# invesalius/invesalius3

Measured on AMD Instinct MI355X. Metric: Mvoxel/s segmentation + Mtriangles/s marching-cubes, 512^3 int16, 1/2/4/8 GPU, higher is better.
Workload: dtype i16; 1 GPU; configs[1]: 512x512x512 int16 per GPU, threshold(226..3071) + 26-neighbour region-grow + marching-cubes(mask@127); global_voxels=134217728, parallelism=z-slab x1, collectives=none, overlap=none

## Files before the change

### include/ivx.h

```cpp
#ifndef IVX_H
#define IVX_H
#include <stddef.h>
#include <stdint.h>

#ifdef __cplusplus
extern "C" {
#endif

#define IVX_OK 0
#define IVX_EINVAL (-1)
#define IVX_ERANGE (-2)
#define IVX_ENOMEM (-3)
#define IVX_EDOM (-4)
#define IVX_EHIP (-5)
#define IVX_ESTALE (-6)

#define IVX_U8 0
#define IVX_I16 1
#define IVX_F64 2
#define IVX_U16 3
#define IVX_F32 4
#define IVX_I32 5
#define IVX_I64 6
#define IVX_I8 7
// ... 366 lines not shown
int ivx_dev_flood_or_planes(const ivx_flood_plan *p, const uint64_t *cand, uint64_t *reached, int64_t z_a,
                            const uint64_t *plane_a, int64_t z_b, const uint64_t *plane_b, void *scratch, int *changed,
                            void *stream);
int ivx_dev_flood_or_planes_dev(const ivx_flood_plan *p, const uint64_t *cand, uint64_t *reached, int64_t z_a,
                                const uint64_t *plane_a, int64_t z_b, const uint64_t *plane_b, void *scratch,
                                uint32_t *changed_dev, void *stream);
int ivx_dev_flood_or_planes_acc(const ivx_flood_plan *p, const uint64_t *cand, uint64_t *reached, int64_t z_a,
                                const uint64_t *plane_a, int64_t z_b, const uint64_t *plane_b, void *scratch,
                                uint32_t *changed_dev, void *stream);
int ivx_dev_flood_apply(const ivx_flood_plan *p, const uint64_t *reached, int dtype, void *target,
                        double fill, void *stream);
int ivx_dev_flood_apply_levels(const ivx_flood_plan *p, const uint64_t *reached, const uint64_t *inside_bits, uint8_t *mask,
                               int v_in, int v_sel, void *stream);
int ivx_dev_mask_from_planes(const ivx_flood_plan *p, const uint64_t *inside_bits, const uint64_t *reached, uint8_t *mask,
                             int v_in, int v_sel, void *stream);
int ivx_dev_flood_apply2(const ivx_flood_plan *p, const uint64_t *reached, uint8_t *out, int fill, uint8_t *mask,
                         int select, void *stream);
int ivx_dev_flood_count(const ivx_flood_plan *p, const uint64_t *reached, int64_t *count, void *stream);
int ivx_flood_edges_bytes(const ivx_flood_plan *p, size_t *nbytes);
int ivx_dev_flood_edges_auto(const ivx_flood_plan *p, const int16_t *data, const uint8_t *out, float pfrac, int fill,
                             uint64_t *edges, void *stream);
int ivx_dev_flood_seed_forced(const ivx_flood_plan *p, const int64_t *seeds_xyz, int64_t nseeds, uint64_t *cand,
                              uint64_t *reached, void *scratch, void *stream);
int ivx_dev_flood_run_edges(const ivx_flood_plan *p, const uint64_t *edges, uint64_t *reached, void *scratch, int *rounds,
                            void *stream);
int ivx_floodfill(int dtype, const void *data, const int64_t shape[3], const int64_t strides[3], int64_t x, int64_t y,
                  int64_t z, double v, int fill, uint8_t *out, const int64_t out_strides[3]);
int ivx_floodfill_auto_threshold(const int16_t *data, const int64_t shape[3], const int64_t strides[3],
                                 const int64_t *seeds_xyz, int64_t nseeds, float pfrac, int fill, uint8_t *out,
                                 const int64_t out_strides[3]);
// ... 257 lines not shown
```

### invesalius3_amd/_lib.py

```python
from __future__ import annotations

import ctypes
import os

import numpy as np

_HERE = os.path.dirname(os.path.abspath(__file__))
LIB_PATH = os.environ.get("IVX_LIB_PATH") or os.path.join(_HERE, "libivx.so")

IVX_OK, IVX_EINVAL, IVX_ERANGE, IVX_ENOMEM, IVX_EDOM, IVX_EHIP, IVX_ESTALE = 0, -1, -2, -3, -4, -5, -6
U8, I16, F64, U16, F32, I32, I64, I8 = 0, 1, 2, 3, 4, 5, 6, 7
DT = {np.dtype(np.uint8): U8, np.dtype(np.int16): I16, np.dtype(np.float64): F64, np.dtype(np.uint16): U16, np.dtype(np.float32): F32, np.dtype(np.int32): I32,
      np.dtype(np.int64): I64}
MIP_MAX, MIP_MIN, MIP_MEAN, MIP_SUM = 0, 1, 2, 3

c_i64 = ctypes.c_int64
c_vp = ctypes.c_void_p


class McParams(ctypes.Structure):
    _fields_ = [
        ("dtype", ctypes.c_int32), ("pad_xy", ctypes.c_int32), ("pad_bottom", ctypes.c_int32),
        ("pad_top", ctypes.c_int32), ("vtk_pz", ctypes.c_int32), ("niso", ctypes.c_int32),
        ("nz", c_i64), ("ny", c_i64), ("nx", c_i64), ("roi_start", c_i64),
        ("pad_value", ctypes.c_double), ("spacing", ctypes.c_double * 3), ("iso", ctypes.c_double * 2),
    ]


class FloodPlan(ctypes.Structure):
    _fields_ = [("dz", c_i64), ("dy", c_i64), ("dx", c_i64), ("wx", c_i64), ("strct_bits", ctypes.c_uint32)]


class VolrenParams(ctypes.Structure):
    _fields_ = [
        ("width", ctypes.c_int32), ("height", ctypes.c_int32), ("mip", ctypes.c_int32), ("shade", ctypes.c_int32),
        ("skip", ctypes.c_int32), ("n_table", ctypes.c_int32), ("out_u8", ctypes.c_int32), ("clip", ctypes.c_int32),
        ("origin", ctypes.c_double * 3), ("du", ctypes.c_double * 3), ("dv", ctypes.c_double * 3),
        ("dir", ctypes.c_double * 3), ("spacing", ctypes.c_double * 3), ("dt", ctypes.c_double),
        ("ambient", ctypes.c_double), ("diffuse", ctypes.c_double), ("specular", ctypes.c_double),
        ("specular_power", ctypes.c_double), ("background", ctypes.c_double * 3), ("clip_normal", ctypes.c_double * 3),
        ("clip_origin", ctypes.c_double * 3),
    ]


ROI_ELLIPSE, ROI_POLYGON, ROI_MAX_POINTS, ROI_RECORD_BYTES = 0, 1, 2048, 40
# ... 18 lines not shown
    i64p = ctypes.POINTER(c_i64)
    for name, args in (("ivx_host_register", [c_vp, sz, u64p]), ("ivx_host_touch", [u64]), ("ivx_host_touch_range", [u64, sz, sz]),
                       ("ivx_host_release", [u64]), ("ivx_host_stats", [u64, u64p]), ("ivx_host_count", [u64p]),
                       ("ivx_host_set_check", [ctypes.c_int]), ("ivx_transfer_stats", [u64p]),
                       ("ivx_upload_strided", [c_vp, c_vp, i64p, i64p, sz]), ("ivx_download_strided", [c_vp, i64p, i64p, c_vp, sz]),
                       ("ivx_image_ranges_bytes", [c_i64, c_i64, c_i64, ctypes.POINTER(sz)]),
                       ("ivx_dev_image_ranges_i16", [c_vp, c_i64, c_i64, c_i64, c_vp, c_vp]),
                       ("ivx_dev_threshold_i16_bits_ranges", [c_vp, c_i64, c_i64, c_i64, ctypes.c_int, ctypes.c_int, c_vp, c_vp, c_vp,
                                                              ctypes.c_int, c_vp]),
                       ("ivx_dev_threshold_i16_plane", [c_vp, c_i64, c_i64, c_i64, ctypes.c_int, ctypes.c_int, c_vp, c_vp]),
                       ("ivx_dev_threshold_i16_plane_ranges", [c_vp, c_i64, c_i64, c_i64, ctypes.c_int, ctypes.c_int, c_vp, c_vp,
                                                               ctypes.c_int, c_vp]),
                       ("ivx_dev_mask_from_planes", [ctypes.POINTER(FloodPlan), c_vp, c_vp, c_vp, ctypes.c_int, ctypes.c_int, c_vp]),
                       ("ivx_dev_flood_candidates_ranges", [ctypes.POINTER(FloodPlan), c_vp, ctypes.c_double, ctypes.c_double, c_vp,
                                                            ctypes.c_int, ctypes.c_double, c_vp, c_vp, c_vp]),
                       ("ivx_dev_image_flip", [c_vp, c_i64, c_i64, c_i64, sz, ctypes.c_int, c_vp]),
                       ("ivx_image_flip", [c_vp, i64p, i64p, sz, ctypes.c_int]),
                       ("ivx_dev_image_swap_axes", [c_vp, c_i64, c_i64, c_i64, sz, ctypes.c_int, ctypes.c_int, c_vp, c_vp]),
                       ("ivx_image_swap_axes", [c_vp, i64p, i64p, sz, ctypes.c_int, ctypes.c_int, c_vp, i64p]),
                       ("ivx_image_tilt_scratch_bytes", [c_i64, c_i64, c_i64, ctypes.POINTER(sz)]),
                       ("ivx_dev_image_fix_gantry_tilt", [c_vp, c_i64, c_i64, c_i64, c_vp, c_vp, sz, c_vp, c_vp]),
                       ("ivx_image_fix_gantry_tilt", [c_vp, i64p, i64p, c_vp, c_vp]),
                       ("ivx_host_zero", [c_vp, sz]), ("ivx_host_register_zero", [c_vp, sz, u64p]),
                       ("ivx_slice_show_tables_bytes", [ctypes.c_int, ctypes.POINTER(sz)]),
                       ("ivx_dev_slice_show", [c_vp, c_i64, c_i64] * 3 + [c_i64, c_i64, c_vp, c_vp, c_vp, c_vp]),
                       ("ivx_slice_show", [c_vp, c_i64, c_i64] * 3 + [c_i64, c_i64, c_vp, c_vp, c_vp]),
                       ("ivx_mask_snapshot_header_bytes", [c_i64, ctypes.POINTER(sz)]),
                       ("ivx_dev_mask_snapshot_scan", [c_vp, c_i64, c_vp, i64p, c_vp]),
                       ("ivx_dev_mask_snapshot_pack", [c_vp, c_i64, c_vp, c_vp, c_i64, c_vp]),
                       ("ivx_dev_mask_snapshot_restore", [c_vp, c_i64, c_vp, c_vp, c_i64, c_i64, c_vp, c_vp]),
# ... 127 lines not shown
```

### invesalius3_amd/csrc/k_flood.hip

```cpp
#include <math.h>
#include <map>
#include <mutex>
#include <stdlib.h>

#include "flood_tiles.h"
#include "words_from_records.h"

namespace {

constexpr int NT = TY * TZ;
constexpr int HY = TY + 2, HZ = TZ + 2;
constexpr int BATCH = 8;
constexpr int SUB = 1;
constexpr unsigned int CLOSED = 0x40u;

template <typename T> __device__ __forceinline__ double as_double(T v) { return (double)v; }

template <typename T, int BAR>
__global__ __launch_bounds__(256) void k_flood_candidates16(const short8_t *__restrict__ data,
                                                            const uint4 *__restrict__ bar, int64_t nchunks, double t0,
                                                            double t1, double fill, uint16_t *__restrict__ cand) {
    const int64_t stride = (int64_t)gridDim.x * blockDim.x;
    const int lo = (int)ceil(t0 < -70000.0 ? -70000.0 : t0), hi = (int)floor(t1 > 70000.0 ? 70000.0 : t1);
    const unsigned fb = (unsigned)(uint8_t)fill;
// ... 946 lines not shown
                auto blend = [&](unsigned int old, unsigned int bits4) {
                    const unsigned int sel = ((bits4 & 1u) * 0xffu) | ((bits4 >> 1 & 1u) * 0xff00u) |
                                             ((bits4 >> 2 & 1u) * 0xff0000u) | ((bits4 >> 3 & 1u) * 0xff000000u);
                    return (old & ~sel) | (f4 & sel);
                };
                v.x = blend(o[u].x, m[u] & 15u);
                v.y = blend(o[u].y, m[u] >> 4 & 15u);
                v.z = blend(o[u].z, m[u] >> 8 & 15u);
                v.w = blend(o[u].w, m[u] >> 12 & 15u);
            }
            out[i0 + u * 256] = v;
        }
    }
}

template <bool ALL>
__global__ __launch_bounds__(256) void k_flood_apply_levels16(const uint16_t *__restrict__ reached, const uint16_t *__restrict__ inside,
                                                              int64_t nchunks, uint4 *__restrict__ out, uint8_t v_in, uint8_t v_sel) {
    const int64_t stride = (int64_t)gridDim.x * 1024;
    const unsigned int in4 = 0x01010101u * v_in, sel4 = 0x01010101u * v_sel;
    for (int64_t i0 = (int64_t)blockIdx.x * 1024 + threadIdx.x; i0 < nchunks; i0 += stride) {
        unsigned int m[4], b[4];
#pragma unroll
        for (int u = 0; u < 4; u++) {
            const int64_t i = i0 + u * 256;
            m[u] = i < nchunks && (!ALL || reached) ? reached[i] : 0u;
            b[u] = i < nchunks ? inside[i] : 0u;
        }
#pragma unroll
        for (int u = 0; u < 4; u++) {
            if (ALL ? i0 + u * 256 >= nchunks : !m[u]) continue;
            auto bytes = [](unsigned int bits4) { return ((bits4 * 0x00204081u) & 0x01010101u) * 0xffu; };
            auto word = [&](unsigned int r4, unsigned int i4) {
// ... 325 lines not shown
template <typename Done>
static int poll_line(volatile unsigned long long *line, long spins, hipStream_t st, Done done, const char *never,
                     unsigned long long *word) {
    for (long n = 0; n < spins; n++) {
        *word = __atomic_load_n((const unsigned long long *)line, __ATOMIC_ACQUIRE);
        if (done(*word)) return IVX_OK;
#if defined(__x86_64__)
        __builtin_ia32_pause();
#endif
    }
    IVX_HIP(hipStreamSynchronize(st));
    *word = __atomic_load_n((const unsigned long long *)line, __ATOMIC_ACQUIRE);
    IVX_REQUIRE(done(*word), IVX_EHIP, "%s", never);
    return IVX_OK;
}
static int flood_run_impl(const ivx_flood_plan *p, const uint64_t *cand, ivx::FloodMode mode, uint64_t *reached, void *scratch_,
                          int *rounds, void *stream, const Fresh *fresh = nullptr) {
    const bool sym = mode == ivx::FLOOD_SYMMETRIC;
    Tiles t;
    int rc = make_tiles(p, &t);
    if (rc) return rc;
    if (rounds) *rounds = 0;
    hipStream_t st = ivx::S(stream);
    GateArm arm = {nullptr, 0u, 0u};
    {
        std::lock_guard<std::mutex> lk(g_gates_mu);
        auto it = g_gates.find(scratch_);
        if (it != g_gates.end()) {
            arm = it->second;
            g_gates.erase(it);
        }
    }
// ... 6 lines not shown
    } gate_guard = {arm, st};
    if (t.ntiles == 0) return IVX_OK;
    const FScratch s = make_fscratch(t);
    char *scr = (char *)scratch_;
    uint8_t *dirty[2] = {(uint8_t *)(scr + s.off_dirty0), (uint8_t *)(scr + s.off_dirty1)};
    unsigned int *cnt = (unsigned int *)(scr + s.off_cnt);
    constexpr int CCL_ESCAPE_ROUNDS = 48;
    if (sym && flood_mode_ccl() && ivx::ccl_supported(p->strct_bits)) {
        if (rounds) *rounds = 1;
        IVX_HIP(hipMemsetAsync(dirty[0], 0, (size_t)t.ntiles, st));
        return ivx::ccl_run(p, cand, reached, scratch_, st);
    }
    int total_rounds = 0;
    unsigned int *list[2] = {(unsigned int *)(scr + s.off_list0), (unsigned int *)(scr + s.off_list1)};
    constexpr int RING = 2 * BATCH;
    static const int ahead = [] {
        const char *e = getenv("IVX_FLOOD_BATCH");
        const int v = e ? atoi(e) : 3;
        return v < 1 ? 1 : (v > BATCH ? BATCH : v);
    }();
    if (coarse_ok(t, mode)) {
        static const Fresh no_seeds = {0, nullptr, 0.0, 0.0, {{}, 0}};
        rc = fresh ? coarse_pass<true>(t, s, scr, cand, reached, *fresh, CNT_CLEARED, st)
                   : coarse_pass<false>(t, s, scr, cand, reached, no_seeds, CNT_CLEARED, st);
        if (rc) return rc;
    } else {
        IVX_REQUIRE(!fresh, IVX_EINVAL, "flood: the fused start needs the coarse pass");
        IVX_HIP(hipMemsetAsync(cnt, 0, CNT_CLEARED * 4, st));
        hipLaunchKernelGGL(k_flood_build_list, dim3((unsigned)ivx::cdiv(t.ntiles, 256)), dim3(256), 0, st, t, dirty[0], list[0], cnt);
        IVX_LAUNCH_CHECK();
    }
    volatile unsigned long long *line = nullptr;
    uint32_t tag = 0;
    if ((rc = ivx::progress_line(st, &line, &tag))) return rc;
    const unsigned grid_max = round_grid_cap(t);
// ... 1 lines not shown
    int64_t queued = 0;
    auto round_kernel = mode == ivx::FLOOD_LINEAR ? k_flood_round_list<2> : mode == ivx::FLOOD_DIRECTED ? k_flood_round_list<1> : k_flood_round_list<0>;
    auto queue_round = [&]() -> int {
        const int r = (int)(queued % RING), cur = (int)(queued & 1);
        const unsigned int tr = (unsigned int)(tag << 24) | (unsigned int)((queued + 1) & 0xffffff);
        hipLaunchKernelGGL(round_kernel, dim3(grid), dim3(NT), 0, st, t, (const unsigned long long *)cand,
                           (unsigned long long *)reached, (const unsigned int *)list[cur], (const unsigned int *)(cnt + r), dirty[cur],
                           dirty[cur ^ 1], list[cur ^ 1], cnt + (r + 1) % RING, cnt + (r + 2) % RING, cnt,
                           (unsigned long long *)line, tr,
                           arm.word, arm.value, arm.below);
        IVX_LAUNCH_CHECK();
        queued++;
        return IVX_OK;
    };
    static const bool trace = getenv("IVX_FLOOD_TRACE") != nullptr;
    int64_t seen = 0;
    for (;;) {
        while (queued < seen + 1 + ahead)
            if ((rc = queue_round())) return rc;
        unsigned long long v = 0;
        rc = poll_line(line, 20000000L, st,
                       [tag, seen](unsigned long long w) { return (uint32_t)(w >> 56) == tag && (int64_t)((w >> 32) & 0xffffffull) > seen; },
                       "flood: the queued rounds never reported", &v);
        if (rc) return rc;
        seen = (int64_t)((v >> 32) & 0xffffffull);
        const unsigned int n_list = (unsigned int)(v & 0xffffffffull);
        if (trace) fprintf(stderr, "ivx flood: round %lld starts with %u of %lld tiles (%lld queued)\n", (long long)seen, n_list,
                           (long long)t.ntiles, (long long)queued);
        if (n_list < arm.below) arm.word = nullptr;
        grid = n_list >= 384u ? grid_max : (n_list >= 96u ? (grid_max < 512u ? grid_max : 512u) : (grid_max < 128u ? grid_max : 128u));
        if (n_list == 0) {
            const unsigned long long u = __atomic_load_n((const unsigned long long *)line + 1, __ATOMIC_ACQUIRE);
            total_rounds = (uint32_t)(u >> 56) == tag ? (int)((u >> 32) & 0xffffffull) : 0;
            break;
        }
        total_rounds = (int)seen;
        if (sym && total_rounds >= CCL_ESCAPE_ROUNDS && ivx::ccl_supported(p->strct_bits)) {
            IVX_HIP(hipMemsetAsync(dirty[0], 0, (size_t)t.ntiles, st));
            IVX_HIP(hipMemsetAsync(dirty[1], 0, (size_t)t.ntiles, st));
            if ((rc = ivx::ccl_run(p, cand, reached, scratch_, st))) return rc;
            total_rounds += 1;
            break;
        }
        IVX_REQUIRE(total_rounds < (1 << 24) - 64, IVX_EHIP, "flood: did not converge");
    }
    if (rounds) *rounds = total_rounds;
    return IVX_OK;
}

int ivx::flood_run(const ivx_flood_plan *p, const uint64_t *planes, ivx::FloodMode mode, uint64_t *reached, void *scratch,
                   int *rounds, void *stream) {
    return flood_run_impl(p, planes, mode, reached, scratch, rounds, stream);
}

extern "C" int ivx_dev_flood_run(const ivx_flood_plan *p, const uint64_t *cand, uint64_t *reached, void *scratch_,
                                 int *rounds, void *stream) {
    return flood_run_impl(p, cand, ivx::FLOOD_SYMMETRIC, reached, scratch_, rounds, stream);
}
static bool fused_start(const Tiles &t, int64_t nseeds) {
    static const bool fused_on = [] {
        const char *e = getenv("IVX_FLOOD_FUSED");
        return !(e && e[0] == '0');
    }();
    return fused_on && nseeds >= 1 && nseeds <= 16 && t.ntiles > 0 && !flood_mode_ccl() && coarse_ok(t, ivx::FLOOD_SYMMETRIC);
}
extern "C" int ivx_dev_flood_grow(const ivx_flood_plan *p, int dtype, const void *data, double t0, double t1,
                                  const int64_t *seeds_xyz, int64_t nseeds, uint64_t *cand, uint64_t *reached, void *scratch_,
                                  int *rounds, void *stream) {
    Tiles t;
    int rc = make_tiles(p, &t);
    if (rc) return rc;
    IVX_REQUIRE(ivx::dtype_size(dtype), IVX_EINVAL, "flood: unsupported dtype %d", dtype);
    for (int64_t n = 0; n < nseeds; n++) {
        const int64_t x = seeds_xyz[3 * n], y = seeds_xyz[3 * n + 1], z = seeds_xyz[3 * n + 2];
        IVX_REQUIRE(x >= 0 && y >= 0 && z >= 0 && x < t.dx && y < t.dy && z < t.dz, IVX_ERANGE,
                    "flood: seed (%lld,%lld,%lld) outside volume (%lld,%lld,%lld) [x,y,z]", (long long)x, (long long)y,
                    (long long)z, (long long)t.dx, (long long)t.dy, (long long)t.dz);
    }
    if (!fused_start(t, nseeds)) {
        if ((rc = ivx_dev_flood_clear(p, reached, scratch_, stream))) return rc;
        if ((rc = ivx_dev_flood_seed(p, dtype, data, t0, t1, seeds_xyz, nseeds, cand, reached, scratch_, stream))) return rc;
        return flood_run_impl(p, cand, ivx::FLOOD_SYMMETRIC, reached, scratch_, rounds, stream);
    }
    ivx::ccl_invalidate(scratch_);
    Fresh f;
    f.dtype = dtype;
    f.data = data;
    f.t0 = t0;
    f.t1 = t1;
    f.sp.n = (int)nseeds;
    for (int64_t n = 0; n < nseeds; n++)
        for (int q = 0; q < 3; q++) f.sp.xyz[n][q] = seeds_xyz[3 * n + q];
    return flood_run_impl(p, cand, ivx::FLOOD_SYMMETRIC, reached, scratch_, rounds, stream, &f);
}
extern "C" int ivx_dev_flood_visits(const ivx_flood_plan *p, const void *scratch_, uint32_t out[2], void *stream) {
    IVX_REQUIRE(scratch_ && out, IVX_EINVAL, "flood_visits: NULL argument");
    Tiles t;
    int rc = make_tiles(p, &t);
    if (rc) return rc;
    out[0] = out[1] = 0u;
    if (t.ntiles == 0) return IVX_OK;
    const FScratch s = make_fscratch(t);
    hipStream_t st = ivx::S(stream);
    unsigned int w[CNT_CLEARED - STATS_AT];
    IVX_HIP(hipMemcpyAsync(w, (const char *)scratch_ + s.off_cnt + STATS_AT * 4, sizeof w, hipMemcpyDeviceToHost, st));
    IVX_HIP(hipStreamSynchronize(st));
    out[0] = w[0];
    for (int k = 0; k < HIST; k++) out[0] += w[HIST_AT - STATS_AT + k];
// ... 11 lines not shown
        const int ct = coarse_lanes(t);
        out[0] = 1;
        out[1] = bk.bxs;
        out[2] = bk.q;
        out[3] = ct;
        out[4] = (int32_t)ivx::cdiv(t.nty * t.ntz, (int64_t)ct);
    }
    out[5] = fused_start(t, nseeds) ? 1 : 0;
    out[6] = (int32_t)round_grid_cap(t);
    out[7] = (int32_t)t.ntiles;
    return IVX_OK;
}

extern "C" int ivx_dev_flood_run_edges(const ivx_flood_plan *p, const uint64_t *edges, uint64_t *reached, void *scratch_,
                                       int *rounds, void *stream) {
    return flood_run_impl(p, edges, ivx::FLOOD_DIRECTED, reached, scratch_, rounds, stream);
}

extern "C" int ivx_flood_edges_bytes(const ivx_flood_plan *p, size_t *nbytes) {
    size_t one;
    int rc = ivx_flood_bits_bytes(p, &one);
    if (rc) return rc;
    *nbytes = 6 * one;
    return IVX_OK;
}

extern "C" int ivx_dev_flood_edges_auto(const ivx_flood_plan *p, const int16_t *data, const uint8_t *out, float pfrac, int fill,
                                        uint64_t *edges, void *stream) {
    Tiles t;
    int rc = make_tiles(p, &t);
    if (rc) return rc;
// ... 96 lines not shown
    case IVX_U8: hipLaunchKernelGGL(k_flood_apply<uint8_t>, dim3(g), dim3(256), 0, st, t, r, (uint8_t *)target, (uint8_t)fill); break;
    case IVX_I16: hipLaunchKernelGGL(k_flood_apply<int16_t>, dim3(g), dim3(256), 0, st, t, r, (int16_t *)target, (int16_t)fill); break;
    case IVX_U16: hipLaunchKernelGGL(k_flood_apply<uint16_t>, dim3(g), dim3(256), 0, st, t, r, (uint16_t *)target, (uint16_t)fill); break;
    case IVX_F64: hipLaunchKernelGGL(k_flood_apply<double>, dim3(g), dim3(256), 0, st, t, r, (double *)target, fill); break;
    default: ivx::set_error("flood: unsupported dtype %d", dtype); return IVX_EINVAL;
    }
    IVX_LAUNCH_CHECK();
    return IVX_OK;
}

extern "C" int ivx_dev_flood_apply_levels(const ivx_flood_plan *p, const uint64_t *reached, const uint64_t *inside_bits, uint8_t *mask,
                                          int v_in, int v_sel, void *stream) {
    Tiles t;
    int rc = make_tiles(p, &t);
    if (rc) return rc;
    IVX_REQUIRE(reached && inside_bits && mask, IVX_EINVAL, "flood_apply_levels: null plane or mask");
    IVX_REQUIRE(t.dx % 64 == 0 && ((uintptr_t)mask & 15) == 0, IVX_EINVAL,
                "flood_apply_levels: rows of whole 64-voxel words and a 16-byte aligned mask only");
    IVX_REQUIRE(v_in >= 0 && v_in <= 255 && v_sel >= 0 && v_sel <= 255, IVX_EINVAL, "flood_apply_levels: levels are bytes");
    const int64_t nchunks = t.dz * t.dy * t.dx / 16;
    if (!nchunks) return IVX_OK;
    const int64_t blocks = ivx::cdiv(nchunks, 1024);
    hipLaunchKernelGGL(k_flood_apply_levels16<false>, dim3((unsigned)(blocks < 16384 ? blocks : 16384)), dim3(256), 0, ivx::S(stream),
                       (const uint16_t *)reached, (const uint16_t *)inside_bits, nchunks, (uint4 *)mask, (uint8_t)v_in, (uint8_t)v_sel);
    IVX_LAUNCH_CHECK();
    return IVX_OK;
}

extern "C" int ivx_dev_mask_from_planes(const ivx_flood_plan *p, const uint64_t *inside_bits, const uint64_t *reached, uint8_t *mask,
                                        int v_in, int v_sel, void *stream) {
    Tiles t;
    int rc = make_tiles(p, &t);
    if (rc) return rc;
    IVX_REQUIRE(inside_bits && mask, IVX_EINVAL, "mask_from_planes: null plane or mask");
    IVX_REQUIRE(t.dx % 64 == 0 && ((uintptr_t)mask & 15) == 0 && (((uintptr_t)inside_bits | (uintptr_t)reached) & 7) == 0, IVX_EINVAL,
                "mask_from_planes: rows of whole 64-voxel words, a 16-byte aligned mask and 8-byte aligned planes only");
    IVX_REQUIRE(v_in >= 0 && v_in <= 255 && v_sel >= 0 && v_sel <= 255, IVX_EINVAL, "mask_from_planes: levels are bytes");
    const int64_t nchunks = t.dz * t.dy * t.dx / 16;
    if (!nchunks) return IVX_OK;
    const int64_t blocks = ivx::cdiv(nchunks, 1024);
    hipLaunchKernelGGL(k_flood_apply_levels16<true>, dim3((unsigned)(blocks < 16384 ? blocks : 16384)), dim3(256), 0, ivx::S(stream),
                       (const uint16_t *)reached, (const uint16_t *)inside_bits, nchunks, (uint4 *)mask, (uint8_t)v_in, (uint8_t)v_sel);
    IVX_LAUNCH_CHECK();
    return IVX_OK;
}

extern "C" int ivx_dev_flood_apply2(const ivx_flood_plan *p, const uint64_t *reached, uint8_t *out, int fill,
                                    uint8_t *mask, int select, void *stream) {
    Tiles t;
    int rc = make_tiles(p, &t);
    if (rc) return rc;
    const int64_t total = t.dz * t.dy * t.wx * 8;
    if (!total) return IVX_OK;
    hipLaunchKernelGGL(k_flood_apply2, dim3(grid_for(total)), dim3(256), 0, ivx::S(stream), t, (const uint8_t *)reached, out,
                       (uint8_t)fill, mask, (uint8_t)select);
    IVX_LAUNCH_CHECK();
    return IVX_OK;
}

// ... 291 lines not shown
```

### invesalius3_amd/device.py

```python
from __future__ import annotations

import ctypes
import os
from typing import NamedTuple, Optional

import numpy as np

from . import _lib as L


class _MaskLevels(NamedTuple):
    v_in: float
    sel: Optional[ctypes.c_void_p]
    v_sel: float

    @property
    def has_second(self):
        return self.sel is not None


class DeviceBuffer:

    def __init__(self, nbytes: int):
        self.nbytes = int(nbytes)
# ... 118 lines not shown
        return e

    class _Span:
        def __init__(self, t, name):
            self.t, self.name = t, name

        def __enter__(self):
            self.e0 = self.t._ev()
            L.check(L.lib().ivx_event_record(self.e0, self.t.stream))

        def __exit__(self, *a):
            e1 = self.t._ev()
            L.check(L.lib().ivx_event_record(e1, self.t.stream))
            self.t.spans.append((self.name, self.e0, e1))

    def span(self, name):
        if self.only is not None and name not in self.only:
            return Timer._OFF
        return Timer._Span(self, name)

    def collect(self) -> dict:
        out = {}
        for name, e0, e1 in self.spans:
            ms = ctypes.c_float(0)
            L.check(L.lib().ivx_event_elapsed_ms(e0, e1, ctypes.byref(ms)))
            out.setdefault(name, []).append(ms.value)
            self._pool += [e0, e1]
        self.spans = []
        return out


class DeviceVolume:
# ... 21 lines not shown
        self._mc_params_cache = {}
        self._stream2 = None
        self._sync_events = []
        self._prefetch = None
        self._gate = None
        self._gate_epoch = 0
        self._gate_armed = False
        self._mbits_version = 0
        self._out_pending = None
        self._mask_pending = False
        self._defer_pays = True
        self._fuse = os.environ.get("IVX_NO_FUSE", "") == ""
        self._apply_levels = os.environ.get("IVX_APPLY_LEVELS", "1") != "0"
        self._use_ranges = os.environ.get("IVX_RANGES", "1") != "0"
        self._mask_defer = os.environ.get("IVX_MASK_DEFER", "1") != "0"
        self._ranges = None
        self._ranges_valid = False
        self.image = TrackedBuffer(self.n * 2, self._image_touched)
        self.mask = TrackedBuffer(self.n, self._mask_touched, self._mask_read)
        self.out_mask = TrackedBuffer(self.n, self._out_touched)
        if image is not None:
            self.image.upload_view(image)
        self.mask.zero(self.stream)
        self.zero_out_mask()
        self.plan = L.FloodPlan(self.dz, self.dy, self.dx, (self.dx + 63) // 64, 0)
        nb, ns = ctypes.c_size_t(0), ctypes.c_size_t(0)
        L.check(L.lib().ivx_flood_bits_bytes(ctypes.byref(self.plan), ctypes.byref(nb)))
        L.check(L.lib().ivx_flood_scratch_bytes(ctypes.byref(self.plan), ctypes.byref(ns)))
        self.cand = DeviceBuffer(nb.value)
        self.reached = DeviceBuffer(nb.value)
# ... 183 lines not shown
    def region_grow(self, seeds_xyz, t0, t1, strct, fill: int = 1, select_value: int | None = 254,
                    image: DeviceBuffer | None = None) -> int:
        lib = L.lib()
        img_ptr = image.ptr if image is not None else self.image.raw
        s3 = np.ascontiguousarray(strct, dtype=np.uint8)
        bits = ctypes.c_uint32(0)
        L.check(lib.ivx_flood_strct_bits(L.ptr(s3), L.i64(s3.shape), ctypes.byref(bits)))
        self.plan.strct_bits = bits.value
        seeds = np.ascontiguousarray(np.array([tuple(s) for s in seeds_xyz], dtype=np.int64).reshape(-1, 3))
        p = ctypes.byref(self.plan)
        st = self.stream
        t0, t1 = float(int(t0)), float(int(t1))
        self._before_flood()
        cand, shared = self._candidate_plane(image, t0, t1, fill)
        rounds = ctypes.c_int(0)
        L.check(lib.ivx_dev_flood_grow(p, L.I16, img_ptr, ctypes.c_double(t0), ctypes.c_double(t1), L.ptr(seeds),
                                       c64(len(seeds)), cand.ptr, self.reached.ptr, self.flood_scratch.ptr,
                                       ctypes.byref(rounds), st), "region_grow")
        self._gate_armed = False
        self._apply_reached(fill, select_value, shared)
        return rounds.value

    def flood_visits(self):
        self._materialize_mask()
        return L.flood_visits(self.plan, self.flood_scratch.ptr, self.stream)

    def _before_flood(self):
        self._materialize_out()
        if self._mask_levels is not None and self._mask_levels[1] is not None:
            self._materialize_mask()
            self._mask_levels = None

    def _candidate_plane(self, image, t0, t1, fill):
        shared = (image is None and self._mbits_valid and self._out_logically_zero() and int(fill) != 0
                  and self._mbits_range == (int(t0), int(t1)))
        if shared:
            return self._mbits, True
        bar, bar_mode = (None, 0) if (self._out_logically_zero() and (int(fill) & 0xff) != 0) else (self.out_mask.raw, 1)
        if image is None and self._use_ranges and self._ranges_valid:
            L.check(L.lib().ivx_dev_flood_candidates_ranges(ctypes.byref(self.plan), self.image.raw, ctypes.c_double(t0),
                                                            ctypes.c_double(t1), bar, bar_mode, ctypes.c_double(fill),
                                                            self._ranges.ptr, self.cand.ptr, self.stream), "flood_candidates_ranges")
            return self.cand, False
        img_ptr = image.ptr if image is not None else self.image.raw
        L.check(L.lib().ivx_dev_flood_candidates(ctypes.byref(self.plan), L.I16, img_ptr, ctypes.c_double(t0),
                                                 ctypes.c_double(t1), bar, bar_mode, ctypes.c_double(fill),
                                                 self.cand.ptr, self.stream))
        return self.cand, False

    def _apply_reached(self, fill, select_value, shared):
        lib, p, st = L.lib(), ctypes.byref(self.plan), self.stream
        if select_value is not None:
            self._mp_cells_valid = False
        defer = self._out_logically_zero() and int(fill) != 0
        levels = select_value is not None and self._mask_levels == (255, None) and self._mbits_valid and self._apply_levels
        if not (defer and levels):
            self._materialize_mask()
        else:
            self._defer_pays = True
        if defer:
            self._out_pending = int(fill)
            if levels and self._mask_pending:
                with self.timer.span("mask_bytes"):
                    L.check(lib.ivx_dev_mask_from_planes(p, self._mbits.ptr, self.reached.ptr, self.mask.raw, 255, int(select_value),
                                                         st), "mask_from_planes")
                self._mask_pending = False
            elif levels:
                L.check(lib.ivx_dev_flood_apply_levels(p, self.reached.ptr, self._mbits.ptr, self.mask.raw, 255, int(select_value), st),
                        "flood_apply_levels")
            elif select_value is not None:
                L.check(lib.ivx_dev_flood_apply(p, self.reached.ptr, L.U8, self.mask.raw, ctypes.c_double(int(select_value)), st))
        elif select_value is not None:
            L.check(lib.ivx_dev_flood_apply2(p, self.reached.ptr, self.out_mask.raw, int(fill), self.mask.raw,
                                             int(select_value), st))
            self._out_bytes_zero = False
        else:
            L.check(lib.ivx_dev_flood_apply(p, self.reached.ptr, L.U8, self.out_mask.raw, ctypes.c_double(fill), st))
            self._out_bytes_zero = False
        if select_value is not None:
            lv = self._mask_levels
            self._mask_levels = (lv[0], int(select_value)) if (lv is not None and lv[1] is None and int(select_value) >= 127
                                                                and self._mbits_valid) else None
        if select_value is not None and self._mbits_valid and not (shared and int(select_value) >= 127):
            self._join_prefetch()
            self._mbits_version += 1
# ... 858 lines not shown
```

Before: 422,600 Mvoxel/s.

## Fuse region-grow with speculative mask write queued behind converging flood rounds

Adds a grow_select entry point that passes the post-flood mask write into the flood loop. Once the active tile list shrinks below a threshold, the loop queues the levels-apply kernel speculatively behind a specific round. That kernel runs only if the round's next list is empty, signals completion through a host-visible line, and lets the host stop polling early. The host look-ahead also becomes adaptive (0 for long lists, 1 otherwise) instead of a fixed 3, while chained callers keep 3. This aims to hide the mask-write launch and host round-trip latency at the end of the flood, at the cost of extra control complexity and possibly wasted no-op launches.

```diff
diff --git a/include/ivx.h b/include/ivx.h
--- a/include/ivx.h
+++ b/include/ivx.h
@@ -404,6 +404,16 @@
                                int v_in, int v_sel, void *stream);
 int ivx_dev_mask_from_planes(const ivx_flood_plan *p, const uint64_t *inside_bits, const uint64_t *reached, uint8_t *mask,
                              int v_in, int v_sel, void *stream);
+enum { IVX_FLOOD_WRITE_NONE = 0, IVX_FLOOD_WRITE_MASK_FROM_PLANES = 1, IVX_FLOOD_WRITE_APPLY_LEVELS = 2, IVX_FLOOD_WRITE_APPLY_U8 = 3 };
+typedef struct ivx_flood_write {
+    int32_t kind, v_in, v_sel, reserved;
+    const uint64_t *inside_bits;
+    uint8_t *mask;
+} ivx_flood_write;
+int ivx_dev_flood_grow_select(const ivx_flood_plan *p, int dtype, const void *data, double t0, double t1,
+                              const int64_t *seeds_xyz, int64_t nseeds, uint64_t *cand, uint64_t *reached, void *scratch,
+                              int *rounds, const ivx_flood_write *write, int look_ahead, void *stream);
+int ivx_flood_look_ahead(int64_t n_list, int32_t *look_ahead);
 int ivx_dev_flood_apply2(const ivx_flood_plan *p, const uint64_t *reached, uint8_t *out, int fill, uint8_t *mask,
                          int select, void *stream);
 int ivx_dev_flood_count(const ivx_flood_plan *p, const uint64_t *reached, int64_t *count, void *stream);
diff --git a/invesalius3_amd/_lib.py b/invesalius3_amd/_lib.py
--- a/invesalius3_amd/_lib.py
+++ b/invesalius3_amd/_lib.py
@@ -29,6 +29,14 @@
 
 class FloodPlan(ctypes.Structure):
     _fields_ = [("dz", c_i64), ("dy", c_i64), ("dx", c_i64), ("wx", c_i64), ("strct_bits", ctypes.c_uint32)]
+
+
+FLOOD_WRITE_NONE, FLOOD_WRITE_MASK_FROM_PLANES, FLOOD_WRITE_APPLY_LEVELS, FLOOD_WRITE_APPLY_U8 = 0, 1, 2, 3
+
+
+class FloodWrite(ctypes.Structure):
+    _fields_ = [("kind", ctypes.c_int32), ("v_in", ctypes.c_int32), ("v_sel", ctypes.c_int32), ("reserved", ctypes.c_int32),
+                ("inside_bits", c_vp), ("mask", c_vp)]
 
 
 class VolrenParams(ctypes.Structure):
@@ -77,6 +85,10 @@
                        ("ivx_dev_mask_from_planes", [ctypes.POINTER(FloodPlan), c_vp, c_vp, c_vp, ctypes.c_int, ctypes.c_int, c_vp]),
                        ("ivx_dev_flood_candidates_ranges", [ctypes.POINTER(FloodPlan), c_vp, ctypes.c_double, ctypes.c_double, c_vp,
                                                             ctypes.c_int, ctypes.c_double, c_vp, c_vp, c_vp]),
+                       ("ivx_dev_flood_grow_select", [ctypes.POINTER(FloodPlan), ctypes.c_int, c_vp, ctypes.c_double, ctypes.c_double,
+                                                      c_vp, c_i64, c_vp, c_vp, c_vp, ctypes.POINTER(ctypes.c_int),
+                                                      ctypes.POINTER(FloodWrite), ctypes.c_int, c_vp]),
+                       ("ivx_flood_look_ahead", [c_i64, ctypes.POINTER(ctypes.c_int32)]),
                        ("ivx_dev_image_flip", [c_vp, c_i64, c_i64, c_i64, sz, ctypes.c_int, c_vp]),
                        ("ivx_image_flip", [c_vp, i64p, i64p, sz, ctypes.c_int]),
                        ("ivx_dev_image_swap_axes", [c_vp, c_i64, c_i64, c_i64, sz, ctypes.c_int, ctypes.c_int, c_vp, c_vp]),
diff --git a/invesalius3_amd/csrc/k_flood.hip b/invesalius3_amd/csrc/k_flood.hip
--- a/invesalius3_amd/csrc/k_flood.hip
+++ b/invesalius3_amd/csrc/k_flood.hip
@@ -984,9 +984,19 @@
     }
 }
 
+struct ApplyWhen {
+    const unsigned int *next_len;
+    unsigned long long *line;
+    unsigned long long report;
+};
 template <bool ALL>
 __global__ __launch_bounds__(256) void k_flood_apply_levels16(const uint16_t *__restrict__ reached, const uint16_t *__restrict__ inside,
-                                                              int64_t nchunks, uint4 *__restrict__ out, uint8_t v_in, uint8_t v_sel) {
+                                                              int64_t nchunks, uint4 *__restrict__ out, uint8_t v_in, uint8_t v_sel,
+                                                              ApplyWhen when) {
+    if (when.next_len) {
+        if (*when.next_len != 0u) return;
+        if (blockIdx.x == 0 && threadIdx.x == 0) __hip_atomic_store(&when.line[2], when.report, __ATOMIC_RELAXED, __HIP_MEMORY_SCOPE_SYSTEM);
+    }
     const int64_t stride = (int64_t)gridDim.x * 1024;
     const unsigned int in4 = 0x01010101u * v_in, sel4 = 0x01010101u * v_sel;
     for (int64_t i0 = (int64_t)blockIdx.x * 1024 + threadIdx.x; i0 < nchunks; i0 += stride) {
@@ -1342,8 +1352,42 @@
     IVX_REQUIRE(done(*word), IVX_EHIP, "%s", never);
     return IVX_OK;
 }
+static int levels_check(const Tiles &t, const uint64_t *reached, const uint64_t *inside_bits, const uint8_t *mask, int v_in, int v_sel,
+                        bool all) {
+    if (all) {
+        IVX_REQUIRE(inside_bits && mask, IVX_EINVAL, "mask_from_planes: null plane or mask");
+        IVX_REQUIRE(t.dx % 64 == 0 && ((uintptr_t)mask & 15) == 0 && (((uintptr_t)inside_bits | (uintptr_t)reached) & 7) == 0, IVX_EINVAL,
+                    "mask_from_planes: rows of whole 64-voxel words, a 16-byte aligned mask and 8-byte aligned planes only");
+        IVX_REQUIRE(v_in >= 0 && v_in <= 255 && v_sel >= 0 && v_sel <= 255, IVX_EINVAL, "mask_from_planes: levels are bytes");
+    } else {
+        IVX_REQUIRE(reached && inside_bits && mask, IVX_EINVAL, "flood_apply_levels: null plane or mask");
+        IVX_REQUIRE(t.dx % 64 == 0 && ((uintptr_t)mask & 15) == 0, IVX_EINVAL,
+                    "flood_apply_levels: rows of whole 64-voxel words and a 16-byte aligned mask only");
+        IVX_REQUIRE(v_in >= 0 && v_in <= 255 && v_sel >= 0 && v_sel <= 255, IVX_EINVAL, "flood_apply_levels: levels are bytes");
+    }
+    return IVX_OK;
+}
+static int launch_levels(const Tiles &t, const uint64_t *reached, const uint64_t *inside, uint8_t *mask, int v_in, int v_sel, bool all,
+                         const ApplyWhen &when, hipStream_t st) {
+    const int64_t nchunks = t.dz * t.dy * t.dx / 16;
+    if (!nchunks) return IVX_OK;
+    const int64_t blocks = ivx::cdiv(nchunks, 1024);
+    auto k = all ? k_flood_apply_levels16<true> : k_flood_apply_levels16<false>;
+    hipLaunchKernelGGL(k, dim3((unsigned)(blocks < 16384 ? blocks : 16384)), dim3(256), 0, st, (const uint16_t *)reached,
+                       (const uint16_t *)inside, nchunks, (uint4 *)mask, (uint8_t)v_in, (uint8_t)v_sel, when);
+    IVX_LAUNCH_CHECK();
+    return IVX_OK;
+}
+constexpr unsigned AHEAD_LONG_LIST = 384u;
+static int default_look_ahead(unsigned n_list) { return n_list >= AHEAD_LONG_LIST ? 0 : 1; }
+struct EarlyWrite {
+    const ivx_flood_write *w;
+    bool written;
+};
+constexpr unsigned EARLY_BELOW = 96u;
+constexpr int EARLY_TRIES = 2;
 static int flood_run_impl(const ivx_flood_plan *p, const uint64_t *cand, ivx::FloodMode mode, uint64_t *reached, void *scratch_,
-                          int *rounds, void *stream, const Fresh *fresh = nullptr) {
+                          int *rounds, void *stream, const Fresh *fresh = nullptr, int look_ahead = -1, EarlyWrite *early = nullptr) {
     const bool sym = mode == ivx::FLOOD_SYMMETRIC;
     Tiles t;
     int rc = make_tiles(p, &t);
@@ -1380,11 +1424,14 @@
     int total_rounds = 0;
     unsigned int *list[2] = {(unsigned int *)(scr + s.off_list0), (unsigned int *)(scr + s.off_list1)};
     constexpr int RING = 2 * BATCH;
-    static const int ahead = [] {
+    static const int env_ahead = [] {
         const char *e = getenv("IVX_FLOOD_BATCH");
-        const int v = e ? atoi(e) : 3;
-        return v < 1 ? 1 : (v > BATCH ? BATCH : v);
+        if (!e || !*e) return -1;
+        const int v = atoi(e);
+        return v < 0 ? 0 : (v > BATCH ? BATCH : v);
     }();
+    const int fixed_ahead = env_ahead >= 0 ? env_ahead : (look_ahead > BATCH ? BATCH : look_ahead);
+    int ahead = fixed_ahead >= 0 ? fixed_ahead : 1;
     if (coarse_ok(t, mode)) {
         static const Fresh no_seeds = {0, nullptr, 0.0, 0.0, {{}, 0}};
         rc = fresh ? coarse_pass<true>(t, s, scr, cand, reached, *fresh, CNT_CLEARED, st)
@@ -1416,26 +1463,64 @@
         return IVX_OK;
     };
     static const bool trace = getenv("IVX_FLOOD_TRACE") != nullptr;
+    static const bool early_on = [] {
+        const char *e = getenv("IVX_FLOOD_EARLY");
+        return !(e && e[0] == '0');
+    }();
+    const bool early_all = early && early->w->kind == IVX_FLOOD_WRITE_MASK_FROM_PLANES;
+    int early_left = 0;
+    if (early_on && early && (early_all || early->w->kind == IVX_FLOOD_WRITE_APPLY_LEVELS) &&
+        levels_check(t, reached, early->w->inside_bits, early->w->mask, early->w->v_in, early->w->v_sel, early_all) == IVX_OK)
+        early_left = EARLY_TRIES;
+    if (early_left) __atomic_store_n((unsigned long long *)line + 2, 0ull, __ATOMIC_RELEASE);
+    int64_t early_at = -1;
+    unsigned long long early_report = 0;
+    bool early_seen = false;
+    unsigned int prev_list = 0xffffffffu;
     int64_t seen = 0;
     for (;;) {
         while (queued < seen + 1 + ahead)
             if ((rc = queue_round())) return rc;
         unsigned long long v = 0;
         rc = poll_line(line, 20000000L, st,
-                       [tag, seen](unsigned long long w) { return (uint32_t)(w >> 56) == tag && (int64_t)((w >> 32) & 0xffffffull) > seen; },
+                       [&](unsigned long long w) {
+                           if (early_at >= 0 && __atomic_load_n((const unsigned long long *)line + 2, __ATOMIC_ACQUIRE) == early_report)
+                               return early_seen = true;
+                           return (uint32_t)(w >> 56) == tag && (int64_t)((w >> 32) & 0xffffffull) > seen;
+                       },
                        "flood: the queued rounds never reported", &v);
         if (rc) return rc;
+        if (early_seen) {
+            const unsigned long long u = __atomic_load_n((const unsigned long long *)line + 1, __ATOMIC_ACQUIRE);
+            total_rounds = (uint32_t)(u >> 56) == tag ? (int)((u >> 32) & 0xffffffull) : 0;
+            early->written = true;
+            if (trace) fprintf(stderr, "ivx flood: the write behind round %lld went ahead (%d rounds with work)\n", (long long)early_at, total_rounds);
+            break;
+        }
         seen = (int64_t)((v >> 32) & 0xffffffull);
         const unsigned int n_list = (unsigned int)(v & 0xffffffffull);
         if (trace) fprintf(stderr, "ivx flood: round %lld starts with %u of %lld tiles (%lld queued)\n", (long long)seen, n_list,
                            (long long)t.ntiles, (long long)queued);
         if (n_list < arm.below) arm.word = nullptr;
         grid = n_list >= 384u ? grid_max : (n_list >= 96u ? (grid_max < 512u ? grid_max : 512u) : (grid_max < 128u ? grid_max : 128u));
+        if (fixed_ahead < 0) ahead = default_look_ahead(n_list);
         if (n_list == 0) {
             const unsigned long long u = __atomic_load_n((const unsigned long long *)line + 1, __ATOMIC_ACQUIRE);
             total_rounds = (uint32_t)(u >> 56) == tag ? (int)((u >> 32) & 0xffffffull) : 0;
+            if (early_at >= 0 && total_rounds <= early_at) early->written = true;
             break;
         }
+        if (early_at >= 0 && seen > early_at) early_at = -1;
+        if (early_left > 0 && early_at < 0 && n_list < EARLY_BELOW && n_list <= prev_list / 2u) {
+            early_at = queued;
+            early_left--;
+            early_report = ((unsigned long long)tag << 56) | ((unsigned long long)(queued & 0xffffff) << 32) | 1ull;
+            if (trace) fprintf(stderr, "ivx flood: write queued behind round %lld\n", (long long)queued);
+            rc = launch_levels(t, reached, early->w->inside_bits, early->w->mask, early->w->v_in, early->w->v_sel, early_all,
+                               ApplyWhen{cnt + queued % RING, (unsigned long long *)line, early_report}, st);
+            if (rc) return rc;
+        }
+        prev_list = n_list;
         total_rounds = (int)seen;
         if (sym && total_rounds >= CCL_ESCAPE_ROUNDS && ivx::ccl_supported(p->strct_bits)) {
             IVX_HIP(hipMemsetAsync(dirty[0], 0, (size_t)t.ntiles, st));
@@ -1450,14 +1535,15 @@
     return IVX_OK;
 }
 
+constexpr int AHEAD_CHAINED = 3;
 int ivx::flood_run(const ivx_flood_plan *p, const uint64_t *planes, ivx::FloodMode mode, uint64_t *reached, void *scratch,
                    int *rounds, void *stream) {
-    return flood_run_impl(p, planes, mode, reached, scratch, rounds, stream);
+    return flood_run_impl(p, planes, mode, reached, scratch, rounds, stream, nullptr, AHEAD_CHAINED);
 }
 
 extern "C" int ivx_dev_flood_run(const ivx_flood_plan *p, const uint64_t *cand, uint64_t *reached, void *scratch_,
                                  int *rounds, void *stream) {
-    return flood_run_impl(p, cand, ivx::FLOOD_SYMMETRIC, reached, scratch_, rounds, stream);
+    return flood_run_impl(p, cand, ivx::FLOOD_SYMMETRIC, reached, scratch_, rounds, stream, nullptr, AHEAD_CHAINED);
 }
 static bool fused_start(const Tiles &t, int64_t nseeds) {
     static const bool fused_on = [] {
@@ -1466,9 +1552,9 @@
     }();
     return fused_on && nseeds >= 1 && nseeds <= 16 && t.ntiles > 0 && !flood_mode_ccl() && coarse_ok(t, ivx::FLOOD_SYMMETRIC);
 }
-extern "C" int ivx_dev_flood_grow(const ivx_flood_plan *p, int dtype, const void *data, double t0, double t1,
-                                  const int64_t *seeds_xyz, int64_t nseeds, uint64_t *cand, uint64_t *reached, void *scratch_,
-                                  int *rounds, void *stream) {
+static int flood_grow_impl(const ivx_flood_plan *p, int dtype, const void *data, double t0, double t1, const int64_t *seeds_xyz,
+                           int64_t nseeds, uint64_t *cand, uint64_t *reached, void *scratch_, int *rounds, void *stream,
+                           int look_ahead, EarlyWrite *early = nullptr) {
     Tiles t;
     int rc = make_tiles(p, &t);
     if (rc) return rc;
@@ -1482,7 +1568,7 @@
     if (!fused_start(t, nseeds)) {
         if ((rc = ivx_dev_flood_clear(p, reached, scratch_, stream))) return rc;
         if ((rc = ivx_dev_flood_seed(p, dtype, data, t0, t1, seeds_xyz, nseeds, cand, reached, scratch_, stream))) return rc;
-        return flood_run_impl(p, cand, ivx::FLOOD_SYMMETRIC, reached, scratch_, rounds, stream);
+        return flood_run_impl(p, cand, ivx::FLOOD_SYMMETRIC, reached, scratch_, rounds, stream, nullptr, look_ahead, early);
     }
     ivx::ccl_invalidate(scratch_);
     Fresh f;
@@ -1493,7 +1579,17 @@
     f.sp.n = (int)nseeds;
     for (int64_t n = 0; n < nseeds; n++)
         for (int q = 0; q < 3; q++) f.sp.xyz[n][q] = seeds_xyz[3 * n + q];
-    return flood_run_impl(p, cand, ivx::FLOOD_SYMMETRIC, reached, scratch_, rounds, stream, &f);
+    return flood_run_impl(p, cand, ivx::FLOOD_SYMMETRIC, reached, scratch_, rounds, stream, &f, look_ahead, early);
+}
+extern "C" int ivx_dev_flood_grow(const ivx_flood_plan *p, int dtype, const void *data, double t0, double t1,
+                                  const int64_t *seeds_xyz, int64_t nseeds, uint64_t *cand, uint64_t *reached, void *scratch_,
+                                  int *rounds, void *stream) {
+    return flood_grow_impl(p, dtype, data, t0, t1, seeds_xyz, nseeds, cand, reached, scratch_, rounds, stream, AHEAD_CHAINED);
+}
+extern "C" int ivx_flood_look_ahead(int64_t n_list, int32_t *look_ahead) {
+    IVX_REQUIRE(look_ahead && n_list >= 0, IVX_EINVAL, "flood_look_ahead: NULL or negative argument");
+    *look_ahead = default_look_ahead(n_list > 0xffffffffll ? 0xffffffffu : (unsigned)n_list);
+    return IVX_OK;
 }
 extern "C" int ivx_dev_flood_visits(const ivx_flood_plan *p, const void *scratch_, uint32_t out[2], void *stream) {
     IVX_REQUIRE(scratch_ && out, IVX_EINVAL, "flood_visits: NULL argument");
@@ -1535,7 +1631,7 @@
 
 extern "C" int ivx_dev_flood_run_edges(const ivx_flood_plan *p, const uint64_t *edges, uint64_t *reached, void *scratch_,
                                        int *rounds, void *stream) {
-    return flood_run_impl(p, edges, ivx::FLOOD_DIRECTED, reached, scratch_, rounds, stream);
+    return flood_run_impl(p, edges, ivx::FLOOD_DIRECTED, reached, scratch_, rounds, stream, nullptr, AHEAD_CHAINED);
 }
 
 extern "C" int ivx_flood_edges_bytes(const ivx_flood_plan *p, size_t *nbytes) {
@@ -1662,17 +1758,8 @@
     Tiles t;
     int rc = make_tiles(p, &t);
     if (rc) return rc;
-    IVX_REQUIRE(reached && inside_bits && mask, IVX_EINVAL, "flood_apply_levels: null plane or mask");
-    IVX_REQUIRE(t.dx % 64 == 0 && ((uintptr_t)mask & 15) == 0, IVX_EINVAL,
-                "flood_apply_levels: rows of whole 64-voxel words and a 16-byte aligned mask only");
-    IVX_REQUIRE(v_in >= 0 && v_in <= 255 && v_sel >= 0 && v_sel <= 255, IVX_EINVAL, "flood_apply_levels: levels are bytes");
-    const int64_t nchunks = t.dz * t.dy * t.dx / 16;
-    if (!nchunks) return IVX_OK;
-    const int64_t blocks = ivx::cdiv(nchunks, 1024);
-    hipLaunchKernelGGL(k_flood_apply_levels16<false>, dim3((unsigned)(blocks < 16384 ? blocks : 16384)), dim3(256), 0, ivx::S(stream),
-                       (const uint16_t *)reached, (const uint16_t *)inside_bits, nchunks, (uint4 *)mask, (uint8_t)v_in, (uint8_t)v_sel);
-    IVX_LAUNCH_CHECK();
-    return IVX_OK;
+    if ((rc = levels_check(t, reached, inside_bits, mask, v_in, v_sel, false))) return rc;
+    return launch_levels(t, reached, inside_bits, mask, v_in, v_sel, false, ApplyWhen{nullptr, nullptr, 0ull}, ivx::S(stream));
 }
 
 extern "C" int ivx_dev_mask_from_planes(const ivx_flood_plan *p, const uint64_t *inside_bits, const uint64_t *reached, uint8_t *mask,
@@ -1680,17 +1767,27 @@
     Tiles t;
     int rc = make_tiles(p, &t);
     if (rc) return rc;
-    IVX_REQUIRE(inside_bits && mask, IVX_EINVAL, "mask_from_planes: null plane or mask");
-    IVX_REQUIRE(t.dx % 64 == 0 && ((uintptr_t)mask & 15) == 0 && (((uintptr_t)inside_bits | (uintptr_t)reached) & 7) == 0, IVX_EINVAL,
-                "mask_from_planes: rows of whole 64-voxel words, a 16-byte aligned mask and 8-byte aligned planes only");
-    IVX_REQUIRE(v_in >= 0 && v_in <= 255 && v_sel >= 0 && v_sel <= 255, IVX_EINVAL, "mask_from_planes: levels are bytes");
-    const int64_t nchunks = t.dz * t.dy * t.dx / 16;
-    if (!nchunks) return IVX_OK;
-    const int64_t blocks = ivx::cdiv(nchunks, 1024);
-    hipLaunchKernelGGL(k_flood_apply_levels16<true>, dim3((unsigned)(blocks < 16384 ? blocks : 16384)), dim3(256), 0, ivx::S(stream),
-                       (const uint16_t *)reached, (const uint16_t *)inside_bits, nchunks, (uint4 *)mask, (uint8_t)v_in, (uint8_t)v_sel);
-    IVX_LAUNCH_CHECK();
-    return IVX_OK;
+    if ((rc = levels_check(t, reached, inside_bits, mask, v_in, v_sel, true))) return rc;
+    return launch_levels(t, reached, inside_bits, mask, v_in, v_sel, true, ApplyWhen{nullptr, nullptr, 0ull}, ivx::S(stream));
+}
+
+extern "C" int ivx_dev_flood_grow_select(const ivx_flood_plan *p, int dtype, const void *data, double t0, double t1,
+                                         const int64_t *seeds_xyz, int64_t nseeds, uint64_t *cand, uint64_t *reached,
+                                         void *scratch_, int *rounds, const ivx_flood_write *write, int look_ahead, void *stream) {
+    IVX_REQUIRE(write && write->kind >= IVX_FLOOD_WRITE_NONE && write->kind <= IVX_FLOOD_WRITE_APPLY_U8, IVX_EINVAL,
+                "flood_grow_select: no write description, or one of an unknown kind");
+    IVX_REQUIRE(write->kind == IVX_FLOOD_WRITE_NONE || write->mask, IVX_EINVAL, "flood_grow_select: the write has no mask");
+    EarlyWrite early = {write, false};
+    int rc = flood_grow_impl(p, dtype, data, t0, t1, seeds_xyz, nseeds, cand, reached, scratch_, rounds, stream, look_ahead, &early);
+    if (rc || early.written) return rc;
+    switch (write->kind) {
+    case IVX_FLOOD_WRITE_MASK_FROM_PLANES:
+        return ivx_dev_mask_from_planes(p, write->inside_bits, reached, write->mask, write->v_in, write->v_sel, stream);
+    case IVX_FLOOD_WRITE_APPLY_LEVELS:
+        return ivx_dev_flood_apply_levels(p, reached, write->inside_bits, write->mask, write->v_in, write->v_sel, stream);
+    case IVX_FLOOD_WRITE_APPLY_U8: return ivx_dev_flood_apply(p, reached, IVX_U8, write->mask, (double)write->v_sel, stream);
+    default: return IVX_OK;
+    }
 }
 
 extern "C" int ivx_dev_flood_apply2(const ivx_flood_plan *p, const uint64_t *reached, uint8_t *out, int fill,
diff --git a/invesalius3_amd/device.py b/invesalius3_amd/device.py
--- a/invesalius3_amd/device.py
+++ b/invesalius3_amd/device.py
@@ -156,8 +156,11 @@
             L.check(L.lib().ivx_event_record(e1, self.t.stream))
             self.t.spans.append((self.name, self.e0, e1))
 
+    def records(self, name) -> bool:
+        return self.only is None or name in self.only
+
     def span(self, name):
-        if self.only is not None and name not in self.only:
+        if not self.records(name):
             return Timer._OFF
         return Timer._Span(self, name)
 
@@ -209,6 +212,8 @@
         self._apply_levels = os.environ.get("IVX_APPLY_LEVELS", "1") != "0"
         self._use_ranges = os.environ.get("IVX_RANGES", "1") != "0"
         self._mask_defer = os.environ.get("IVX_MASK_DEFER", "1") != "0"
+        self._select = os.environ.get("IVX_FLOOD_SELECT", "1") != "0"
+        self._look_ahead = -1
         self._ranges = None
         self._ranges_valid = False
         self.image = TrackedBuffer(self.n * 2, self._image_touched)
@@ -422,11 +427,17 @@
         self._before_flood()
         cand, shared = self._candidate_plane(image, t0, t1, fill)
         rounds = ctypes.c_int(0)
-        L.check(lib.ivx_dev_flood_grow(p, L.I16, img_ptr, ctypes.c_double(t0), ctypes.c_double(t1), L.ptr(seeds),
-                                       c64(len(seeds)), cand.ptr, self.reached.ptr, self.flood_scratch.ptr,
-                                       ctypes.byref(rounds), st), "region_grow")
+        write = self._flood_write(fill, select_value) if self._select else None
+        if write is not None:
+            L.check(lib.ivx_dev_flood_grow_select(p, L.I16, img_ptr, ctypes.c_double(t0), ctypes.c_double(t1), L.ptr(seeds),
+                                                  c64(len(seeds)), cand.ptr, self.reached.ptr, self.flood_scratch.ptr,
+                                                  ctypes.byref(rounds), ctypes.byref(write), int(self._look_ahead), st), "region_grow")
+        else:
+            L.check(lib.ivx_dev_flood_grow(p, L.I16, img_ptr, ctypes.c_double(t0), ctypes.c_double(t1), L.ptr(seeds),
+                                           c64(len(seeds)), cand.ptr, self.reached.ptr, self.flood_scratch.ptr,
+                                           ctypes.byref(rounds), st), "region_grow")
         self._gate_armed = False
-        self._apply_reached(fill, select_value, shared)
+        self._apply_reached(fill, select_value, shared, queued=write is not None)
         return rounds.value
 
     def flood_visits(self):
@@ -456,27 +467,44 @@
                                                  self.cand.ptr, self.stream))
         return self.cand, False
 
-    def _apply_reached(self, fill, select_value, shared):
+    def _write_kind(self, fill, select_value):
+        if not (self._out_logically_zero() and int(fill) != 0):
+            return None
+        if select_value is not None and self._mask_levels == (255, None) and self._mbits_valid and self._apply_levels:
+            return L.FLOOD_WRITE_MASK_FROM_PLANES if self._mask_pending else L.FLOOD_WRITE_APPLY_LEVELS
+        return L.FLOOD_WRITE_APPLY_U8 if select_value is not None else L.FLOOD_WRITE_NONE
+
+    def _flood_write(self, fill, select_value):
+        kind = self._write_kind(fill, select_value)
+        if kind is None or (kind == L.FLOOD_WRITE_MASK_FROM_PLANES and self.timer.records("mask_bytes")):
+            return None
+        if kind == L.FLOOD_WRITE_APPLY_U8:
+            self._materialize_mask()
+        return L.FloodWrite(kind=kind, v_in=255, v_sel=int(select_value) if select_value is not None else 0,
+                            inside_bits=self._mbits.ptr.value, mask=self.mask.raw.value)
+
+    def _apply_reached(self, fill, select_value, shared, queued=False):
         lib, p, st = L.lib(), ctypes.byref(self.plan), self.stream
         if select_value is not None:
             self._mp_cells_valid = False
-        defer = self._out_logically_zero() and int(fill) != 0
-        levels = select_value is not None and self._mask_levels == (255, None) and self._mbits_valid and self._apply_levels
-        if not (defer and levels):
+        kind = self._write_kind(fill, select_value)
+        assert kind is not None or not queued
+        if kind not in (L.FLOOD_WRITE_MASK_FROM_PLANES, L.FLOOD_WRITE_APPLY_LEVELS):
             self._materialize_mask()
         else:
             self._defer_pays = True
-        if defer:
+        if kind is not None:
             self._out_pending = int(fill)
-            if levels and self._mask_pending:
-                with self.timer.span("mask_bytes"):
-                    L.check(lib.ivx_dev_mask_from_planes(p, self._mbits.ptr, self.reached.ptr, self.mask.raw, 255, int(select_value),
-                                                         st), "mask_from_planes")
+            if kind == L.FLOOD_WRITE_MASK_FROM_PLANES:
+                if not queued:
+                    with self.timer.span("mask_bytes"):
+                        L.check(lib.ivx_dev_mask_from_planes(p, self._mbits.ptr, self.reached.ptr, self.mask.raw, 255,
+                                                             int(select_value), st), "mask_from_planes")
                 self._mask_pending = False
-            elif levels:
+            elif kind == L.FLOOD_WRITE_APPLY_LEVELS and not queued:
                 L.check(lib.ivx_dev_flood_apply_levels(p, self.reached.ptr, self._mbits.ptr, self.mask.raw, 255, int(select_value), st),
                         "flood_apply_levels")
-            elif select_value is not None:
+            elif kind == L.FLOOD_WRITE_APPLY_U8 and not queued:
                 L.check(lib.ivx_dev_flood_apply(p, self.reached.ptr, L.U8, self.mask.raw, ctypes.c_double(int(select_value)), st))
         elif select_value is not None:
             L.check(lib.ivx_dev_flood_apply2(p, self.reached.ptr, self.out_mask.raw, int(fill), self.mask.raw,
```

New measurement: 430,200 Mvoxel/s, median of 6. 1.02x the previous value.
